# JanEGerken/HEAL-SWIN

Hardware: AMD Instinct MI355X
Metric: images/sec fwd+bwd, HEAL-SWIN nside=256 seg, batch=8 at 1/2/4/8 MI355X (higher is better)
Workload: dtype bf16

## Files before the change

### heal_swin_amd/_lib.py

```python
import ctypes
import os

import numpy as np

_PKG = os.path.dirname(os.path.abspath(__file__))
LIB_PATH = os.path.join(_PKG, "lib", "libhealswin.so")

HS_F32, HS_BF16 = 0, 1
HS_F64 = 3
HS_PRED_LABELS, HS_PRED_ROWS16 = 2, 4
HS_ENSEMBLE_PROB, HS_ENSEMBLE_LOGIT = 0, 1
HS_ATTN_COSINE = 1
HS_ATTN_FORCE_VALU = 2
HS_ATTN_RESIDUAL = 4
HS_ATTN_OVERWRITE_GRADS = 8
HS_EPI_BIAS, HS_EPI_GELU, HS_EPI_DGELU, HS_EPI_RESID = 0, 1, 2, 3
HS_ACC_DEFER = 2
HS_MLP_NORM_AFTER = 16
HS_U8, HS_I32, HS_I64 = 8, 9, 10
HS_FLAT_PATCH_ROWS, HS_FLAT_PIXEL_ROWS, HS_FLAT_IMAGE = 0, 1, 2
HS_DEPTH_L1, HS_DEPTH_L2, HS_DEPTH_HUBER, HS_DEPTH_LOGVAR = 0, 1, 2, 3
HS_DT_NONE, HS_DT_LOG, HS_DT_INV = 0, 1, 2
HS_DT_ZERO_BKG, HS_DT_1000_BKG, HS_DT_AFFINE, HS_DT_INVERSE = 1, 2, 4, 8
HS_DEPTH_STATS_WORDS = 15
HS_HISTOGRAM_MAX_BINS = 4096

c_i64 = ctypes.c_int64
c_int = ctypes.c_int
c_uint = ctypes.c_uint
c_ptr = ctypes.c_void_p
c_float = ctypes.c_float


class WgradProblem(ctypes.Structure):
    _fields_ = [("dy", c_ptr), ("x", c_ptr), ("dw", c_ptr), ("dbias", c_ptr), ("n_out", c_int), ("k_in", c_int), ("accumulate", c_int),
                ("gelu_x", c_int)]


def wgrad_problems(members):
# ... 380 lines not shown
```

### heal_swin_amd/csrc/gemm_nt.hip

```cpp
#include <cstdlib>

#include "hs_gelu.h"

namespace hs {
HS_DEFINE_SEED_EPOCH_SETTER(set_seed_epoch_gemm_nt)

#ifdef HS_GEMM_TRACE
#define HS_GEMM_TRACE_PARAM uint64_t* trace;
constexpr int kTraceCap = 240;
static uint64_t* g_trace = nullptr;
extern "C" int hs_gemm_nt_set_trace(void* buf) {
    g_trace = (uint64_t*)buf;
    return 0;
}
template <typename Params>
void trace_attach(Params& p) {
    p.trace = g_trace;
}
constexpr int trace_lds(int used, int nw) { return used + nw * kTraceCap * 8 <= 163840 ? nw * kTraceCap * 8 : 0; }
struct Trace {
    uint64_t* out;
    bool on;
    int n = 0, nw, wave, lane;
    uint32_t base;
// ... 22 lines not shown
    }
};
#else
#define HS_GEMM_TRACE_PARAM
template <typename Params>
void trace_attach(Params&) {}
constexpr int trace_lds(int, int) { return 0; }
struct Trace {
    template <typename Params>
    __device__ __forceinline__ Trace(const Params&, bool, uint32_t, int, int, int) {}
    __device__ __forceinline__ void operator()(int) const {}
    __device__ __forceinline__ void flush() const {}
};
#endif

namespace {

typedef unsigned int u32x2 __attribute__((__vector_size__(8)));
typedef unsigned int u32x4v __attribute__((__vector_size__(16)));

constexpr int kStoreAux = 2;
constexpr int kInAux = 2;
enum { EPI_BIAS = 0, EPI_GELU = 1, EPI_DGELU = 2, EPI_RESID = 3 };
constexpr int64_t kMaxRecords = 0x7FFFFE00;

struct GemmParams {
    const uint16_t *a, *b;
    int64_t lda, ldb;
    int k;
    const uint16_t *a2, *b2;
    int64_t lda2, ldb2;
    int k2;
    const float* bias;
    uint16_t* c;
    uint16_t* aux;
    int64_t m;
    int n;
    int tiles_n, tiles, per_xcd, blocks_per_xcd;
    float drop_p;
    uint64_t seed;
    HS_GEMM_TRACE_PARAM
};

template <int BM_, int BN_, int WM_, int WN_, int NSTAGE_, bool ALIAS_, int WGS_PER_CU_>
struct TileTraits {
    static constexpr int BM = BM_, BN = BN_, WM = WM_, WN = WN_, NSTAGE = NSTAGE_, WGS_PER_CU = WGS_PER_CU_;
    static constexpr bool ALIAS = ALIAS_;
    static constexpr int NW = WM * WN;
    static constexpr int TM = BM / WM / 32, TN = BN / WN / 32;
    static constexpr int AB = BM * 128, BB = BN * 128, STAGE = AB + BB;
    static constexpr int AHEAD = NSTAGE - 1;
    static_assert(TN == 2 && (TM == 2 || TM == 4), "the kernel is written for wave tiles of 64 columns and 64 or 128 rows");
    static_assert(!ALIAS || NW * 4096 <= STAGE, "patches do not fit a stage buffer");
    static_assert(BN * 4 <= 1024, "a bias slot holds one 1-KB DMA piece");

    static constexpr bool has_in(int epi) { return epi == EPI_DGELU || epi == EPI_RESID; }
    static constexpr bool ring(int epi) { return has_in(epi) && ALIAS && TM == 4 && STAGE >= NW * 8192; }
    static constexpr bool lbias(int epi) { return ALIAS && epi != EPI_DGELU; }
    static constexpr int NSLOT = NSTAGE + 1;
    static constexpr int PATCH_OFF = NSTAGE * STAGE;
    static constexpr int BIAS_OFF = NSTAGE * STAGE + (ALIAS ? 0 : NW * 4096);
    static constexpr int bias_lds(int epi) { return lbias(epi) ? NSLOT * 1024 : 0; }
    static constexpr int trace_off(int epi) { return BIAS_OFF + bias_lds(epi); }
    static constexpr int lds_bytes(int epi) { return trace_off(epi) + trace_lds(trace_off(epi), NW); }
};
using Tile1 = TileTraits<128, 128, 2, 2, 2, false, 2>;
using Tile2 = TileTraits<256, 128, 4, 2, 3, true, 1>;
using Tile3 = TileTraits<256, 256, 2, 4, 2, true, 1>;

constexpr int epi_younger_ops(int tm, int i) {
    const int stores = i < 2 ? i : 1;
    const int last_d = i + 1 < tm - 1 ? i + 1 : tm - 1;
    return 4 * (stores + (last_d - i));
}

template <int OFF>
__device__ __forceinline__ u32x4 lds_read_b128(uint32_t addr) {
    u32x4 v;
    asm volatile("ds_read_b128 %0, %1 offset:%2" : "=v"(v) : "v"(addr), "n"(OFF));
    return v;
}
constexpr int next_in_ring(int x, int n) { return x + 1 == n ? 0 : x + 1; }
__device__ __forceinline__ u32x2 pack_bf16x4(f32x2 lo, f32x2 hi) { return u32x2{pack_bf16x2(lo.x, lo.y), pack_bf16x2(hi.x, hi.y)}; }
__device__ __forceinline__ __amdgpu_buffer_rsrc_t clamped_rsrc(const void* ptr, int64_t bytes) {
    bytes = bytes > kMaxRecords ? kMaxRecords : bytes;
    return __builtin_amdgcn_make_buffer_rsrc((void*)ptr, 0, (int)bytes, 0x00020000);
}
template <int LATER, int EPI_OPS>
__device__ __forceinline__ void wait_pieces_behind() {
    static_assert(LATER + EPI_OPS <= 63, "vmcnt immediate");
    asm volatile("s_waitcnt vmcnt(%0)" ::"n"(LATER + EPI_OPS) : "memory");
}

template <int N_, int LDS_, bool SC>
struct Operand {
    static constexpr int N = N_, LDS = LDS_, J = SC ? 4 : N;
// ... 11 lines not shown
        }
    }
    __device__ __forceinline__ void retarget(const uint16_t* base, int64_t ld, int64_t row0, int64_t rows, int kseg) {
        rsrc = clamped_rsrc(base + row0 * ld, (rows - row0 - 1) * ld * 2 + kseg);
#pragma unroll
        for (int j = 0; j < J; ++j) off[j] = row[j] * ((int)ld * 2) + col[j];
        ld32 = (int)ld * 64;
    }
    __device__ __forceinline__ void issue(unsigned char* stage, int wave, int q, int kb, int kseg) const {
        lds_void* dst = (lds_void*)(stage + LDS + (wave * N + q) * 1024);
        if constexpr (SC) {
            __builtin_amdgcn_raw_ptr_buffer_load_lds(rsrc, dst, 16, (uint32_t)off[q % J], kb + (q >> 2) * ld32, 0, 0);
        } else {
            const uint32_t voff = kb + col[q] < kseg ? (uint32_t)(off[q] + kb) : kOob;
            __builtin_amdgcn_raw_ptr_buffer_load_lds(rsrc, dst, 16, voff, 0, 0, 0);
        }
    }
};
__device__ __forceinline__ uint32_t frag_addr(uint32_t lds_base, int r, int half) {
    const int R = r >> 1;
    return lds_base + R * 256 + (((((r & 1) << 3) + half) ^ (R & 15)) << 4);
}

template <typename Tile, int EPI, bool DROP, bool FAST>
__global__ void __launch_bounds__(Tile::NW * 64, 2) gemm_nt_kernel(GemmParams p) {
#if defined(__HIP_DEVICE_COMPILE__)
    constexpr int BM = Tile::BM, BN = Tile::BN, WM = Tile::WM, WN = Tile::WN, NW = Tile::NW, TM = Tile::TM, TN = Tile::TN;
    constexpr int NSTAGE = Tile::NSTAGE, AHEAD = Tile::AHEAD, NSLOT = Tile::NSLOT, STAGE = Tile::STAGE, BIAS_OFF = Tile::BIAS_OFF;
    constexpr bool ALIAS = Tile::ALIAS, HAS_IN = Tile::has_in(EPI), RING = Tile::ring(EPI), LBIAS = Tile::lbias(EPI);
    constexpr int IW = FAST ? NW / 2 : NW;
    using OperandA = Operand<Tile::AB / 1024 / IW, 0, FAST>;
    using OperandB = Operand<Tile::BB / 1024 / IW, Tile::AB, FAST>;
    constexpr int PIECES = OperandA::N + OperandB::N;
    static_assert(Tile::lds_bytes(EPI) <= 163840, "LDS of one workgroup exceeds 160 KB");
    __shared__ __attribute__((aligned(16))) unsigned char smem[Tile::lds_bytes(EPI)];

    const int tid = threadIdx.x, lane = tid & 63, half = lane >> 5, l31 = lane & 31;
    const int wave = __builtin_amdgcn_readfirstlane(tid >> 6);
    const int wm = wave / WN, wn = wave % WN;

    const int xcd = blockIdx.x & 7, lb = blockIdx.x >> 3;
    const int id_end = min((xcd + 1) * p.per_xcd, p.tiles);
    const int id0 = xcd * p.per_xcd + lb;
    if (id0 >= id_end) return;
    const int nk1 = (p.k + 63) >> 6, nk2 = (p.k2 + 63) >> 6, nk = nk1 + nk2;
    struct Origin {
        int64_t m0;
        int n0;
    };
    auto tile_origin = [&](int id) {
        const int tm = id / p.tiles_n, tn = id - tm * p.tiles_n;
        return Origin{(int64_t)tm * BM, tn * BN};
// ... 86 lines not shown
            constexpr int ks = decltype(ks_c)::value;
            constexpr int rest = PIECES - ks * PQ, cnt = rest < 0 ? 0 : rest < PQ ? rest : PQ;
            wait_frags(ks_c, Int<(ks < 3 ? TM + TN : 0)>{});
            mma(ks_c, Int<ks * PQ>{}, Int<cnt>{});
            if constexpr (ks + 2 < 4) read_frags(Int<ks + 2>{});
        });
    };

    const uint32_t own_rel = wave * 4096 + l31 * 128 + 8 * half;
    const uint32_t own_out_rel = wave * 4096 + l31 * 128 + 8 * (half ^ ((l31 >> 3) & 1));
    const uint32_t row_rel = wave * 4096 + (lane >> 3) * 128 + (((lane & 7) ^ (lane >> 3)) << 4);
    const bool second_half = ((half ^ (lane & (p.n >> 2))) & 1) != 0;
    auto epilogue = [&](int id, int buf_done, int slot_c) {
        const uint32_t patch_off = ALIAS ? buf_done * STAGE : Tile::PATCH_OFF;
        TR(10);
        if (ALIAS) __builtin_amdgcn_s_barrier();
        TR(11);
        const Origin o = tile_origin(id);
        const int64_t m0 = o.m0;
        const int n2 = p.n * 2;
        const int64_t cbytes = (p.m - m0) * (int64_t)n2;
        const __amdgpu_buffer_rsrc_t rc = clamped_rsrc(p.c + m0 * p.n, p.c ? cbytes : 0);
        const __amdgpu_buffer_rsrc_t rx = clamped_rsrc(p.aux + m0 * p.n, p.aux ? cbytes : 0);
        const ElemRng rng(p.drop_p, p.seed);
        const bool wide = RING || (p.n & 7) == 0;
        const int ncol0 = o.n0 + wn * (BN / WN);
        auto col_of = [&](int j, int g) { return ncol0 + j * 32 + 4 * half + 8 * g; };
        float4 bias4[TN][4];
        const uint32_t baddr = lds0 + BIAS_OFF + slot_c * 1024 + (wn * (BN / WN) + 4 * half) * 4;
        auto lds_bias = [&](int j, float4 (&b)[4]) {
            u32x4 bq[4];
#pragma unroll
            for (int g = 0; g < 4; ++g) asm volatile("ds_read_b128 %0, %1" : "=v"(bq[g]) : "v"(baddr + (j * 32 + 8 * g) * 4));
            asm volatile("s_waitcnt lgkmcnt(0)" : "+v"(bq[0]), "+v"(bq[1]), "+v"(bq[2]), "+v"(bq[3]));
#pragma unroll
            for (int g = 0; g < 4; ++g) b[g] = __builtin_bit_cast(float4, bq[g]);
        };
        if constexpr (!LBIAS) {
#pragma unroll
            for (int j = 0; j < TN; ++j)
#pragma unroll
                for (int g = 0; g < 4; ++g) {
                    const int n = col_of(j, g);
                    bias4[j][g] = (EPI != EPI_DGELU && p.bias && n < p.n) ? *(const float4*)(p.bias + n) : make_float4(0.f, 0.f, 0.f, 0.f);
                }
        }
        const int rl_col = ncol0 + (lane & 7) * 8;
        const uint32_t rl_voff = rl_col < p.n ? (uint32_t)((lane >> 3) * n2 + rl_col * 2) : kOob;
        auto row_soff = [&](int i, int t) -> int { return (wm * (BM / WM) + i * 32 + 8 * t) * n2; };
        const int in_col = ncol0 + (((lane & 7) ^ (lane >> 3)) << 3);
        const uint32_t in_voff = in_col < p.n ? (uint32_t)((lane >> 3) * n2 + in_col * 2) : kOob;
        auto request_in = [&](int i) {
            unsigned char* base = smem + patch_off + (i & 1) * (NW * 4096) + wave * 4096;
#pragma unroll
            for (int t = 0; t < 4; ++t)
                __builtin_amdgcn_raw_ptr_buffer_load_lds(rx, (lds_void*)(base + t * 1024), 16, in_voff, row_soff(i, t), 0, kInAux);
        };
        if constexpr (RING) {
            request_in(0);
            request_in(1);
        }
#pragma unroll
        for (int i = 0; i < TM; ++i) {
            const int ml = wm * (BM / WM) + i * 32 + l31;
            auto direct_off = [&](int j, int g) { return col_of(j, g) < p.n ? (uint32_t)(ml * n2 + col_of(j, g) * 2) : kOob; };
            const uint32_t pbase = lds0 + patch_off + (RING ? (i & 1) * (NW * 4096) : 0);
            const uint32_t own_addr = pbase + own_rel, row_addr = pbase + row_rel, own_out = pbase + own_out_rel;
            u32x2 xin[TN][4];
            if (HAS_IN) {
                if (wide) {
                    if constexpr (RING) {
                        static_for<TM>([&](auto b) {
                            if (i == b) asm volatile("s_waitcnt vmcnt(%0)" ::"n"(epi_younger_ops(TM, b)) : "memory");
                        });
                    } else {
                        u32x4 rws[4];
#pragma unroll
                        for (int t = 0; t < 4; ++t)
                            rws[t] = __builtin_bit_cast(u32x4, __builtin_amdgcn_raw_buffer_load_b128(rx, rl_voff, row_soff(i, t), 0));
                        asm volatile("ds_write_b128 %0, %1" ::"v"(row_addr), "v"(rws[0]) : "memory");
                        asm volatile("ds_write_b128 %0, %1 offset:1024" ::"v"(row_addr), "v"(rws[1]) : "memory");
                        asm volatile("ds_write_b128 %0, %1 offset:2048" ::"v"(row_addr), "v"(rws[2]) : "memory");
                        asm volatile("ds_write_b128 %0, %1 offset:3072" ::"v"(row_addr), "v"(rws[3]) : "memory");
                    }
#pragma unroll
                    for (int j = 0; j < TN; ++j)
#pragma unroll
                        for (int g = 0; g < 4; ++g)
                            asm volatile("ds_read_b64 %0, %1" : "=v"(xin[j][g]) : "v"(own_addr + (((4 * j + g) ^ (l31 & 7)) << 4)));
                    asm volatile("s_waitcnt lgkmcnt(0)"
                                 : "+v"(xin[0][0]), "+v"(xin[0][1]), "+v"(xin[0][2]), "+v"(xin[0][3]), "+v"(xin[1][0]),
                                   "+v"(xin[1][1]), "+v"(xin[1][2]), "+v"(xin[1][3]));
                } else {
#pragma unroll
                    for (int j = 0; j < TN; ++j)
#pragma unroll
                        for (int g = 0; g < 4; ++g) xin[j][g] = __builtin_amdgcn_raw_buffer_load_b64(rx, direct_off(j, g), 0, 0);
                }
            }
            auto chunk_key = [&](int j, int g) { return rng.chunk_key((uint64_t)((m0 + ml) * p.n + col_of(j, g)) >> 3); };
            auto keep2 = [&](uint32_t ck, int t) {
                const uint32_t hh = ElemRng::pair_bits(ck, ElemRng::half_mult(second_half, t));
                return f32x2{rng.keep_lo(hh), rng.keep_hi(hh)};
            };
            u32x2 o1[TN][4], o2[TN][4];
#pragma unroll
            for (int j = 0; j < TN; ++j) {
                if constexpr (LBIAS) lds_bias(j, bias4[j]);
#pragma unroll
                for (int g = 0; g < 4; ++g) {
                    f32x16& a16 = acc[j][i];
                    f32x2 v[2] = {f32x2{a16[4 * g], a16[4 * g + 1]} + f32x2{bias4[j][g].x, bias4[j][g].y},
                                  f32x2{a16[4 * g + 2], a16[4 * g + 3]} + f32x2{bias4[j][g].z, bias4[j][g].w}};
                    uint32_t ck = 0;
                    if (DROP) ck = chunk_key(j, g);
// ... 40 lines not shown
                            }
                            o2[j][g] = pack_bf16x4(v[2 * gg], v[2 * gg + 1]);
#pragma unroll
                            for (int r = 0; r < 4; ++r) a16[4 * g + r] = 0.f;
                        }
                    }
            };
            TR(20);
            auto emit = [&](const __amdgpu_buffer_rsrc_t& rs, const u32x2 (&o)[TN][4]) {
                if (wide) {
#pragma unroll
                    for (int j = 0; j < TN; ++j)
#pragma unroll
                        for (int g = 0; g < 4; ++g)
                            asm volatile("ds_write_b64 %0, %1" ::"v"(own_out + (((4 * j + g) ^ (l31 & 7)) << 4)), "v"(o[j][g]) : "memory");
                    u32x4 rws[4];
                    asm volatile("ds_read_b128 %0, %1" : "=v"(rws[0]) : "v"(row_addr));
                    asm volatile("ds_read2_b64 %0, %1 offset0:129 offset1:128" : "=v"(rws[1]) : "v"(row_addr));
                    asm volatile("ds_read_b128 %0, %1 offset:2048" : "=v"(rws[2]) : "v"(row_addr));
                    asm volatile("ds_read2_b64 %0, %1 offset0:129 offset1:128" : "=v"(rws[3]) : "v"(row_addr + 2048));
                    asm volatile("s_waitcnt lgkmcnt(0)" : "+v"(rws[0]), "+v"(rws[1]), "+v"(rws[2]), "+v"(rws[3]));
                    TR(22);
#pragma unroll
                    for (int t = 0; t < 4; ++t)
                        __builtin_amdgcn_raw_buffer_store_b128(__builtin_bit_cast(u32x4v, rws[t]), rs, rl_voff, row_soff(i, t), kStoreAux);
                    asm volatile("s_nop 0" ::"v"(rws[0]), "v"(rws[1]), "v"(rws[2]), "v"(rws[3]));
                } else {
#pragma unroll
                    for (int j = 0; j < TN; ++j)
#pragma unroll
                        for (int g = 0; g < 4; ++g) __builtin_amdgcn_raw_buffer_store_b64(o[j][g], rs, direct_off(j, g), 0, kStoreAux);
                }
            };
            if (EPI == EPI_GELU) {
                if (NW == 8 && wave >= NW / 2) {
                    make_o2();
                    emit(rx, o2);
                    TR(21);
                    __builtin_amdgcn_sched_barrier(0);
                    if (p.c) emit(rc, o1);
                } else {
                    if (p.c) emit(rc, o1);
                    TR(21);
                    __builtin_amdgcn_sched_barrier(0);
                    make_o2();
                    emit(rx, o2);
                }
            } else {
                emit(rc, o1);
            }
            if constexpr (RING) {
                if (i + 2 < TM) request_in(i + 2);
            }
            TR(12 + i);
        }
    };

    const int stride = p.blocks_per_xcd;
    int id_i = id0, ks_i = 0;
    int id_c = id0, ks_c = 0;
    int slot_c = 0;
    auto advance_issue = [&]() {
        ++ks_i;
        if (ks_i == nk) {
            ks_i = 0;
            id_i += stride;
            if (id_i < id_end) retarget(id_i, nk1 == 0, true);
        } else if (ks_i == nk1) {
            retarget(id_i, true, false);
        }
    };
    auto kb_of = [&](int ks) { return (ks >= nk1 ? ks - nk1 : ks) * 128; };
    retarget(id_i, false, true);
    int issued = 0;
#pragma unroll
    for (int q = 0; q < AHEAD; ++q) {
        if (id_i < id_end) {
            issue_pieces(kb_of(ks_i), q, Int<0>{}, Int<PIECES>{});
            advance_issue();
            ++issued;
        }
    }
    int buf = 0, buf_free = AHEAD;
    bool drained = false;
    constexpr int LATER = (AHEAD - 1) * PIECES;
    constexpr int kEpiOps = TM * 4;
    TR(0);
    while (true) {
        TR(3);
        if (IW < NW && wave >= IW) {
        } else if (AHEAD > 1 && issued == AHEAD && !drained)
            wait_pieces_behind<LATER, 0>();
        else if (drained && issued == AHEAD)
            wait_pieces_behind<LATER, kEpiOps>();
        else if (drained && issued == 1)
            wait_pieces_behind<0, kEpiOps>();
        else
            wait_pieces_behind<0, 0>();
        drained = false;
        TR(1);
        __builtin_amdgcn_s_barrier();
        TR(2);
        const bool more = id_i < id_end;
        const bool last = ks_c + 1 == nk;
        compute(buf, more, kb_of(ks_i), buf_free);
        --issued;
        if (more) {
            advance_issue();
            ++issued;
        }
        const int buf_done = buf;
        buf = next_in_ring(buf, NSTAGE);
        buf_free = next_in_ring(buf_free, NSTAGE);
        if (last) {
            epilogue(id_c, buf_done, slot_c);
            slot_c = next_in_ring(slot_c, NSLOT);
            drained = true;
            ks_c = 0;
            id_c += stride;
            if (id_c >= id_end) break;
        } else {
            ++ks_c;
        }
    }
    TR.flush();
#endif
}

template <typename Tile, bool FAST>
int launch_tile(GemmParams& p, int epi, hipStream_t s) {
    const int tiles_m = (int)((p.m + Tile::BM - 1) / Tile::BM);
    p.tiles_n = (p.n + Tile::BN - 1) / Tile::BN;
    const int64_t tiles = (int64_t)tiles_m * p.tiles_n;
    if (tiles > 0x7fffffff) return fail(HS_ERR_UNSUPPORTED, "too many output tiles");
    p.tiles = (int)tiles;
    p.per_xcd = (p.tiles + 7) / 8;
    const int resident = usable_cus_per_xcd() * Tile::WGS_PER_CU;
    p.blocks_per_xcd = p.per_xcd < resident ? p.per_xcd : resident;
    const dim3 grid((unsigned)(8 * p.blocks_per_xcd)), block(Tile::NW * 64);
    using Kernel = void (*)(GemmParams);
    static constexpr Kernel kKernels[4][2] = {
        {gemm_nt_kernel<Tile, EPI_BIAS, false, FAST>, gemm_nt_kernel<Tile, EPI_BIAS, false, FAST>},
        {gemm_nt_kernel<Tile, EPI_GELU, false, FAST>, gemm_nt_kernel<Tile, EPI_GELU, true, FAST>},
        {gemm_nt_kernel<Tile, EPI_DGELU, false, FAST>, gemm_nt_kernel<Tile, EPI_DGELU, true, FAST>},
        {gemm_nt_kernel<Tile, EPI_RESID, false, FAST>, gemm_nt_kernel<Tile, EPI_RESID, false, FAST>}};
    hipLaunchKernelGGL(kKernels[epi][p.drop_p > 0.f], grid, block, 0, s, p);
    HS_LAUNCH_CHECK("gemm_nt");
    return HS_OK;
}

}

int gemm_nt_check_shape(const char* who, int64_t lda, int64_t ldb, int k, int64_t lda2, int64_t ldb2, int k2, int64_t m, int n) {
    HS_CHECK_ARG(m > 0 && n > 0 && k > 0 && k2 >= 0, "%s: empty shape", who);
    if (k % 8 || k2 % 8 || lda % 8 || ldb % 8 || (k2 && (lda2 % 8 || ldb2 % 8)) || n % 4)
        return fail(HS_ERR_UNSUPPORTED, "%s: k, k2 and the row strides must be multiples of 8, n a multiple of 4", who);
    if (lda * 2 * 256 > kMaxRecords || ldb * 2 * 256 > kMaxRecords || (int64_t)n * 2 * 256 > kMaxRecords)
        return fail(HS_ERR_UNSUPPORTED, "%s: row stride too large", who);
    if (((m + 127) / 128) * (((int64_t)n + 127) / 128) > 0x7fffffff) return fail(HS_ERR_UNSUPPORTED, "%s: too many output tiles", who);
    return HS_OK;
}

int gemm_nt_tile_variant(int forced, int64_t m, int n, int k, int k2, int epilogue) {
    int variant = forced;
    if (!variant) {
        const int64_t tiles2 = ((m + 255) / 256) * ((n + 127) / 128), tiles3 = ((m + 255) / 256) * ((n + 255) / 256);
        if (tiles2 < 256)
            variant = 1;
        else if ((epilogue == EPI_GELU || epilogue == EPI_DGELU) ? n >= 512 : (n >= 1024 && k + k2 >= 512))
// ... 1 lines not shown
        else if (n >= 256 && tiles3 >= 768 && k % 64 == 0 && k2 % 64 == 0)
            variant = 3;
        else
            variant = 2;
    }
    if (variant == 3 && (epilogue == EPI_DGELU || epilogue == EPI_RESID) && n % 8) variant = 2;
    return variant == 2 || variant == 3 ? variant : 1;
}

}

namespace {
int g_tile_variant = 0;
}

extern "C" {

int hs_gemm_nt_set_tile(int variant) {
    g_tile_variant = variant;
    return HS_OK;
}

int hs_gemm_nt_tile_variant(int64_t m, int n, int k, int k2, int epilogue) {
    return hs::gemm_nt_tile_variant(g_tile_variant, m, n, k, k2, epilogue);
}

int hs_gemm_nt(const void* a, int64_t lda, const void* b, int64_t ldb, int k, const void* a2, int64_t lda2, const void* b2,
               int64_t ldb2, int k2, const float* bias, void* c, void* aux, int64_t m, int n, int epilogue, float drop_p,
               uint64_t seed, int dtype, void* stream) {
    using namespace hs;
    HS_CHECK_ARG(dtype == HS_BF16, "hs_gemm_nt: bf16 activations only (fp32 runs use the library GEMM)");
    HS_CHECK_ARG(a && b && m > 0 && n > 0 && k > 0, "hs_gemm_nt: null operand or empty shape");
    HS_CHECK_ARG(epilogue >= EPI_BIAS && epilogue <= EPI_RESID, "hs_gemm_nt: unknown epilogue %d", epilogue);
    HS_CHECK_ARG(k2 == 0 || (a2 && b2 && k2 > 0), "hs_gemm_nt: second segment needs a2, b2, k2 > 0");
    HS_CHECK_ARG(c || (epilogue == EPI_GELU && aux), "hs_gemm_nt: no output");
    HS_CHECK_ARG(epilogue == EPI_BIAS || aux, "hs_gemm_nt: this epilogue needs aux");
    HS_CHECK_ARG(drop_p >= 0.f && drop_p <= 1.f, "hs_gemm_nt: drop_p must be in [0, 1]");
    HS_CHECK_ALIGNED("hs_gemm_nt", 16, a, b, a2, b2, bias, c, aux);
    if (int st = gemm_nt_check_shape("hs_gemm_nt", lda, ldb, k, lda2, ldb2, k2, m, n)) return st;
    GemmParams p{};
    p.a = (const uint16_t*)a; p.b = (const uint16_t*)b; p.lda = lda; p.ldb = ldb; p.k = k;
    p.a2 = (const uint16_t*)a2; p.b2 = (const uint16_t*)b2; p.lda2 = lda2; p.ldb2 = ldb2; p.k2 = k2;
    p.bias = bias; p.c = (uint16_t*)c; p.aux = (uint16_t*)aux; p.m = m; p.n = n;
    p.drop_p = drop_p; p.seed = seed;
    trace_attach(p);
    hipStream_t st = (hipStream_t)stream;
    const bool fast = k % 64 == 0 && k2 % 64 == 0;
    switch (gemm_nt_tile_variant(g_tile_variant, m, n, k, k2, epilogue)) {
        case 2: return fast ? launch_tile<Tile2, true>(p, epilogue, st) : launch_tile<Tile2, false>(p, epilogue, st);
        case 3: return fast ? launch_tile<Tile3, true>(p, epilogue, st) : launch_tile<Tile3, false>(p, epilogue, st);
        default: return launch_tile<Tile1, false>(p, epilogue, st);
    }
}

}
```

### heal_swin_amd/ops/gemm.py

```python
import math
import os

import torch

from .. import _lib
from .._lib import check, lib, ptr, stream_ptr
from . import runtime
from .runtime import RT, _aligned, _cast_param, _defer_flag, _defer_keep, _require_gpu, _sink_buffer, _timed


OWN_GEMM = os.environ.get("HS_OWN_GEMM", "auto")


OWN_GELU_MAX_K = 4096
OWN_DGELU_MAX_K = 1024
OWN_BIAS_MAX_K = 0


class GemmTuner:
    MIN_FLOP = 1 << 33

    def __init__(self):
        self.picks = {}
        self.trials = {}
# ... 54 lines not shown
    if epi == _lib.HS_EPI_DGELU:
        return kk <= OWN_DGELU_MAX_K
    if epi == _lib.HS_EPI_GELU:
        return kk <= OWN_GELU_MAX_K
    if OWN_BIAS_MAX_K > 0:
        return kk <= OWN_BIAS_MAX_K
    if GEMM_TUNE and m is not None and k2 == 0 and torch.cuda.is_available():
        pick = GEMM_TUNER.pick(int(m), n, kk, torch.device("cuda", torch.cuda.current_device()))
        if pick is not None:
            return pick
    return kk <= 128 or n <= 128 or (n <= 256 and kk <= 256)


RESID_DGRAD_OWN = True


def own_gemm_legal(n, k, dtype):
    return dtype == torch.bfloat16 and OWN_GEMM != "0" and k % 8 == 0 and n % 8 == 0 and n >= 16


RESID_EPILOGUE = True


def gemm_nt(a2d, w, bias=None, epi=0, aux=None, a2=None, w2=None, want_c=True, drop_p=0.0, seed=0):
    w, w2, bias = _aligned(w), _aligned(w2), _aligned(bias)
    if epi != _lib.HS_EPI_GELU:
        aux = _aligned(aux)
    m, k = a2d.shape
    n = w.shape[0]
    assert a2d.stride(1) == 1 and w.stride(1) == 1 and a2d.dtype == torch.bfloat16 and w.dtype == torch.bfloat16
    c = torch.empty((m, n), dtype=torch.bfloat16, device=a2d.device) if want_c else None
    if epi == _lib.HS_EPI_GELU:
        aux = torch.empty((m, n), dtype=torch.bfloat16, device=a2d.device)
    k2 = 0 if a2 is None else a2.shape[1]
    if bias is not None and bias.dtype != torch.float32:
        bias = bias.float()
    with _timed(f"hs_gemm_nt epi={epi} m={m} n={n} k={k + k2}", a2d.device, 2 * (m * (k + k2) + n * (k + k2) + m * n * (2 if (epi and want_c) else 1)), 2 * m * n * (k + k2)):
        check(lib.hs_gemm_nt(ptr(a2d), a2d.stride(0), ptr(w), w.stride(0), k, ptr(a2), 0 if a2 is None else a2.stride(0), ptr(w2),
                             0 if w2 is None else w2.stride(0), k2, ptr(bias), ptr(c), ptr(aux), m, n, epi, float(drop_p), int(seed),
                             _lib.HS_BF16, stream_ptr(a2d.device)), "hs_gemm_nt")
    return c, aux


def _lib_tag(kind, m, n, k):
    return f"lib {kind} m={m} n={n} k={k}"


FP32_GEMM = os.environ.get("HS_FP32_GEMM", "bf16x3")
_BF16X3_MIN = 160
_SPLIT_MEMO = []
_MM_OUT_DTYPE = [None]


def _bf16x3_ok(x, n=None, k=None):
    ok = FP32_GEMM == "bf16x3" and x.dtype == torch.float32 and x.is_cuda and x.shape[-1] % 8 == 0
    ok = ok and (n is None or n * k >= _BF16X3_MIN * (n + k))
    if ok and _MM_OUT_DTYPE[0] is None:
        _probe_mm_out_dtype(x.device)
    return ok and _MM_OUT_DTYPE[0] is not False


def _probe_mm_out_dtype(device):
# ... 396 lines not shown
```

### heal_swin_amd/ops/mlp_branch.py

```python
import os

import torch

from .. import _lib
from .._lib import check, lib, ptr, stream_ptr
from .runtime import RT, _aligned, _cast_param, _defer_flag, _defer_keep, _draw_seed, _extras, _f32, _require_gpu, _timed
from .norm import _norm_param_grads, _norm_param_result
from .gemm import (_Split, _bf16x3_ok, _cast_param_t, _input_grad, _lib_linear, _lib_linear_resid, _lib_matmul, _param_grads, lib_resid_ok, _split_of, gemm_nt, own_gemm_legal, own_gemm_ok)


class MlpFn(torch.autograd.Function):

    @staticmethod
    def forward(ctx, x, w1, b1, w2, b2, drop_p, seed, passthrough, residual=None):
        _require_gpu(x, w1, b1, w2, b2, residual)
        c_in, hid = w1.shape[1], w1.shape[0]
        x2 = x.reshape(-1, c_in)
        if not x2.is_contiguous():
            x2 = x2.contiguous()
        dt = x.dtype
        x3 = a3 = None
        w1c, w2c = _cast_param(w1, dt), _cast_param(w2, dt)
        need_grad = any(ctx.needs_input_grad[:5])
        if own_gemm_ok(_lib.HS_EPI_GELU, hid, c_in, dt):
            h, a = gemm_nt(x2, w1c, b1, _lib.HS_EPI_GELU, want_c=need_grad, drop_p=drop_p, seed=seed)
        else:
            h = _lib_linear(x2, w1c, None if b1 is None else _cast_param(b1, dt))
            x3 = _split_of(x2)
            if _bf16x3_ok(h, w2.shape[0], hid) and w2c.dtype == torch.float32 and w2.shape[0] % 8 == 0 and hid % 8 == 0:
                h = _aligned(h)
                a3 = torch.empty((h.shape[0], 3 * hid), dtype=torch.bfloat16, device=h.device)
                check(lib.hs_gelu_split3(None, ptr(h), ptr(a3), h.shape[0], hid, float(drop_p), int(seed), stream_ptr(h.device)),
                      "hs_gelu_split3")
                a = _Split(a3, hid)
            else:
                a = torch.empty_like(h)
                check(lib.hs_gelu_fwd(ptr(h), ptr(a), h.numel(), float(drop_p), int(seed), _lib.dtype_code(dt), stream_ptr(h.device)),
                      "hs_gelu_fwd")
        ctx.has_residual = residual is not None
        res2 = None
        if residual is not None:
            res2 = residual.reshape(-1, w2.shape[0])
            res2 = res2 if res2.is_contiguous() else res2.contiguous()
        lib_res = res2 is not None and lib_resid_ok(w2.shape[0], hid, dt) and not own_gemm_ok(_lib.HS_EPI_BIAS, w2.shape[0], hid, dt, m=x2.shape[0])
        if lib_res:
            y = _lib_linear_resid(a, w2c, None if b2 is None else _cast_param(b2, dt), res2)
        elif res2 is not None and own_gemm_legal(w2.shape[0], hid, dt):
            y = gemm_nt(a, w2c, b2, _lib.HS_EPI_RESID, aux=res2)[0]
# ... 9 lines not shown
        assert not isinstance(a, _Split)
        ctx.save_for_backward(None if x3 is not None else x2, h, None if a3 is not None else a, w1, w2)
        ctx.biases = (b1, b2)
        ctx.casts = (w1c if w1c.dtype != w1.dtype else None, w2c if w2c.dtype != w2.dtype else None)
        ctx.cast_cache = RT.cast_cache
        ctx.meta = (float(drop_p), int(seed), x.shape)
        ctx.splits = (x3, a3)
        y = y.view(x.shape[:-1] + (w2.shape[0],))
        return (y, x.view_as(x)) if passthrough else y

    @staticmethod
    def backward(ctx, dy, dx_res=None):
        x2, h, a, w1, w2 = ctx.saved_tensors
        b1, b2 = ctx.biases
        w1c, w2c = ctx.casts
        p, seed, xshape = ctx.meta
        if dy is None:
            return dx_res, None, None, None, None, None, None, None, None
        c_out, hid, c_in = w2.shape[0], w1.shape[0], w1.shape[1]
        dy2 = dy.reshape(-1, c_out)
        if not dy2.is_contiguous():
            dy2 = dy2.contiguous()
        dt = dy2.dtype
        if own_gemm_ok(_lib.HS_EPI_DGELU, hid, c_out, dt):
            dh = gemm_nt(dy2, _cast_param_t(w2, dt, ctx.cast_cache), None, _lib.HS_EPI_DGELU, aux=h, drop_p=p, seed=seed)[0]
        else:
            da = _lib_matmul(dy2, w2c if (w2c is not None and w2c.dtype == dt) else w2.to(dt))
            if _bf16x3_ok(da, c_in, hid) and w1.dtype == torch.float32 and c_in % 8 == 0 and hid % 8 == 0:
                dh3 = torch.empty((h.shape[0], 3 * hid), dtype=torch.bfloat16, device=h.device)
                check(lib.hs_gelu_split3(ptr(_aligned(da)), ptr(_aligned(h)), ptr(dh3), h.shape[0], hid, p, seed, stream_ptr(h.device)), "hs_gelu_split3")
                dh = _Split(dh3, hid)
            else:
                dh = torch.empty_like(h)
                check(lib.hs_gelu_bwd(ptr(da), ptr(h), ptr(dh), h.numel(), p, seed, _lib.dtype_code(dt), stream_ptr(h.device)), "hs_gelu_bwd")
            del da
        dx = None
        if ctx.needs_input_grad[0]:
            dx = _input_grad(dh, w1, w1c, None if dx_res is None else dx_res.reshape(-1, c_in), ctx.cast_cache).reshape(xshape)
        ctx.casts = ctx.cast_cache = None
        (x3, a3), ctx.splits = ctx.splits, (None, None)
        dw2, db2 = _param_grads(dy2, a, w2, b2, ctx.needs_input_grad[3], b2 is not None and ctx.needs_input_grad[4], a3)
        dw1, db1 = _param_grads(dh, x2, w1, b1, ctx.needs_input_grad[1], b1 is not None and ctx.needs_input_grad[2], x3)
        return dx, dw1, db1, dw2, db2, None, None, None, (dy if ctx.has_residual else None)


def mlp(x, w1, b1, w2, b2, drop_p=0.0, seed=None, passthrough=False, residual=None):
    if drop_p > 0.0 and seed is None:
        seed = _draw_seed()
# ... 122 lines not shown
```

### include/healswin.h

```cpp
#ifndef HEALSWIN_H
#define HEALSWIN_H

#include <stdint.h>

#ifdef __cplusplus
extern "C" {
#endif

typedef enum {
    HS_OK = 0,
    HS_ERR_INVALID_ARG = 1,
    HS_ERR_UNSUPPORTED = 2,
    HS_ERR_HIP = 3,
    HS_ERR_NOT_PERMUTATION = 4,
    HS_ERR_MISALIGNED = 5
} hs_status;

typedef enum { HS_F32 = 0, HS_BF16 = 1 } hs_dtype;

#define HS_ATTN_COSINE 1u
#define HS_ATTN_FORCE_VALU 2u
#define HS_ATTN_RESIDUAL 4u
#define HS_ATTN_OVERWRITE_GRADS 8u

// ... 205 lines not shown
                              int64_t n_tokens, int channels, int num_heads, int window_size, unsigned flags, int dtype,
                              void* stream);

int hs_window_attn_module_fwd_train(const void* x, void* out, void* xn_out, float* mean_out, float* rstd_out, void* qkv_out,
                                    void* attn_out, float* lse_out, const void* qkv_w, const float* qkv_b, const void* proj_w,
                                    const float* proj_b, const float* ln_gamma, const float* ln_beta, const float* bias,
                                    const float* head_scale, const int32_t* idx, int64_t roll, const uint8_t* labels,
                                    const float* norm2_gamma, const float* norm2_beta, void* n2_out, float* mean2_out, float* rstd2_out,
                                    int batch, int64_t n_tokens, int channels, int num_heads, int window_size, unsigned flags, int dtype,
                                    void* stream);

int64_t hs_window_attn_module_bwd_chain_workspace(int batch, int64_t n_tokens, int channels, int num_heads, int window_size);
int hs_window_attn_module_bwd_chain(const void* dout, const void* x, const void* xn, const float* mean, const float* rstd, const void* qkv,
                              const void* attn_out, const float* lse, const void* qkv_w_t, const void* proj_w_t, const float* ln_gamma,
                              const float* bias, const float* head_scale, const int32_t* idx, int64_t roll, const uint8_t* labels,
                              void* dx, float* dqkv_w, float* dqkv_b, float* dproj_w, float* dproj_b, float* dln_gamma, float* dln_beta,
                              float* dbias, float* dhead_scale, float* workspace, int accumulate, int batch, int64_t n_tokens, int channels,
                              int num_heads, int window_size, unsigned flags, int dtype, void* stream);

#define HS_EPI_BIAS 0
#define HS_EPI_GELU 1
#define HS_EPI_DGELU 2
#define HS_EPI_RESID 3
int hs_gemm_nt(const void* a, int64_t lda, const void* b, int64_t ldb, int k, const void* a2, int64_t lda2, const void* b2,
               int64_t ldb2, int k2, const float* bias, void* c, void* aux, int64_t m, int n, int epilogue, float drop_p,
               uint64_t seed, int dtype, void* stream);
int hs_gemm_nt_set_tile(int variant);
int hs_gemm_nt_tile_variant(int64_t m, int n, int k, int k2, int epilogue);

int hs_lib_gemm_supported(void);
int hs_lib_gemm_set_supported(int on);
int hs_lib_gemm_nt(const void* a, const void* w, const void* bias, int bias_dtype, const void* c, void* d, int64_t m, int n, int k,
                   void* stream);
int hs_lib_gemm_pick(int64_t m, int n, int k, int has_c, int* index, int* solution, char* name, int name_len);
int hs_lib_gemm_set_pick(int64_t m, int n, int k, int has_c, int index);

int hs_pix2ang_nest(int nside, int64_t first, int64_t count, double* theta, double* phi);
int hs_sample_bilinear_u8(const void* img, int batch, int channels, int height, int width, const double* rx, const double* ry,
                          int64_t n, void* out, void* stream);
int hs_sample_mask_u8(const void* mask, int batch, int height, int width, const double* rx, const double* ry, int64_t n,
                      int background, void* out, void* stream);

typedef struct hs_fisheye_camera {
    double k[8];
    double cx_offset, cy_offset, aspect_ratio;
    int poly_order, width, height;
// ... 223 lines not shown
```

Before: 58.82.

## Store MLP hidden activations as per-tile records for the GELU-backward GEMM

Adds an HS_EPI_RECORDS mode for the 256x256 tile. The forward GELU GEMM writes the pre-activation h in a tile-blocked record layout that follows the per-wave fragment order, so each lane stores contiguous 16-byte chunks. The backward DGELU GEMM reads those records straight into LDS and skips the swizzled per-row segment reads and the stride-dependent addressing. It is on by default through HS_MLP_RECORDS. In exchange, h becomes an opaque padded buffer tied to the forward and backward GEMMs both picking tile variant 3.

```diff
diff --git a/heal_swin_amd/_lib.py b/heal_swin_amd/_lib.py
--- a/heal_swin_amd/_lib.py
+++ b/heal_swin_amd/_lib.py
@@ -15,6 +15,7 @@
 HS_ATTN_RESIDUAL = 4
 HS_ATTN_OVERWRITE_GRADS = 8
 HS_EPI_BIAS, HS_EPI_GELU, HS_EPI_DGELU, HS_EPI_RESID = 0, 1, 2, 3
+HS_EPI_RECORDS = 0x100
 HS_ACC_DEFER = 2
 HS_MLP_NORM_AFTER = 16
 HS_U8, HS_I32, HS_I64 = 8, 9, 10
diff --git a/heal_swin_amd/csrc/gemm_nt.hip b/heal_swin_amd/csrc/gemm_nt.hip
--- a/heal_swin_amd/csrc/gemm_nt.hip
+++ b/heal_swin_amd/csrc/gemm_nt.hip
@@ -68,6 +68,8 @@
 constexpr int kStoreAux = 2;
 constexpr int kInAux = 2;
 enum { EPI_BIAS = 0, EPI_GELU = 1, EPI_DGELU = 2, EPI_RESID = 3 };
+enum { EPI_CODE_MASK = 0xff, EPI_RECORDS = 0x100 };
+constexpr int kRowOps = 4;
 constexpr int64_t kMaxRecords = 0x7FFFFE00;
 
 struct GemmParams {
@@ -103,6 +105,8 @@
     static constexpr bool has_in(int epi) { return epi == EPI_DGELU || epi == EPI_RESID; }
     static constexpr bool ring(int epi) { return has_in(epi) && ALIAS && TM == 4 && STAGE >= NW * 8192; }
     static constexpr bool lbias(int epi) { return ALIAS && epi != EPI_DGELU; }
+    static constexpr bool records(int epi) { return ALIAS && TM == 4 && NW == 8 && (epi == EPI_GELU || epi == EPI_DGELU); }
+    static constexpr int RECORD = BM * BN;
     static constexpr int NSLOT = NSTAGE + 1;
     static constexpr int PATCH_OFF = NSTAGE * STAGE;
     static constexpr int BIAS_OFF = NSTAGE * STAGE + (ALIAS ? 0 : NW * 4096);
@@ -117,7 +121,7 @@
 constexpr int epi_younger_ops(int tm, int i) {
     const int stores = i < 2 ? i : 1;
     const int last_d = i + 1 < tm - 1 ? i + 1 : tm - 1;
-    return 4 * (stores + (last_d - i));
+    return kRowOps * (stores + (last_d - i));
 }
 
 template <int OFF>
@@ -175,12 +179,13 @@
     return lds_base + R * 256 + (((((r & 1) << 3) + half) ^ (R & 15)) << 4);
 }
 
-template <typename Tile, int EPI, bool DROP, bool FAST>
+template <typename Tile, int EPI, bool DROP, bool FAST, bool REC = false>
 __global__ void __launch_bounds__(Tile::NW * 64, 2) gemm_nt_kernel(GemmParams p) {
 #if defined(__HIP_DEVICE_COMPILE__)
     constexpr int BM = Tile::BM, BN = Tile::BN, WM = Tile::WM, WN = Tile::WN, NW = Tile::NW, TM = Tile::TM, TN = Tile::TN;
     constexpr int NSTAGE = Tile::NSTAGE, AHEAD = Tile::AHEAD, NSLOT = Tile::NSLOT, STAGE = Tile::STAGE, BIAS_OFF = Tile::BIAS_OFF;
     constexpr bool ALIAS = Tile::ALIAS, HAS_IN = Tile::has_in(EPI), RING = Tile::ring(EPI), LBIAS = Tile::lbias(EPI);
+    static_assert(!REC || (Tile::records(EPI) && (EPI == EPI_GELU || RING)), "records: the 256 x 256 tile's GELU / GELU' epilogues");
     constexpr int IW = FAST ? NW / 2 : NW;
     using OperandA = Operand<Tile::AB / 1024 / IW, 0, FAST>;
     using OperandB = Operand<Tile::BB / 1024 / IW, Tile::AB, FAST>;
@@ -313,6 +318,9 @@
         const int64_t cbytes = (p.m - m0) * (int64_t)n2;
         const __amdgpu_buffer_rsrc_t rc = clamped_rsrc(p.c + m0 * p.n, p.c ? cbytes : 0);
         const __amdgpu_buffer_rsrc_t rx = clamped_rsrc(p.aux + m0 * p.n, p.aux ? cbytes : 0);
+        uint16_t* const hrec = EPI == EPI_GELU ? p.c : p.aux;
+        const __amdgpu_buffer_rsrc_t rrec = clamped_rsrc(hrec + (REC ? (int64_t)id * Tile::RECORD : 0), REC && hrec ? Tile::RECORD * 2 : 0);
+        auto rec_soff = [&](int i, int t) -> int { return wave * (TM * kRowOps * 1024) + (i * kRowOps + t) * 1024; };
         const ElemRng rng(p.drop_p, p.seed);
         const bool wide = RING || (p.n & 7) == 0;
         const int ncol0 = o.n0 + wn * (BN / WN);
@@ -344,8 +352,10 @@
         auto request_in = [&](int i) {
             unsigned char* base = smem + patch_off + (i & 1) * (NW * 4096) + wave * 4096;
 #pragma unroll
-            for (int t = 0; t < 4; ++t)
-                __builtin_amdgcn_raw_ptr_buffer_load_lds(rx, (lds_void*)(base + t * 1024), 16, in_voff, row_soff(i, t), 0, kInAux);
+            for (int t = 0; t < kRowOps; ++t) {
+                if constexpr (REC) __builtin_amdgcn_raw_ptr_buffer_load_lds(rrec, (lds_void*)(base + t * 1024), 16, lane * 16, rec_soff(i, t), 0, kInAux);
+                else __builtin_amdgcn_raw_ptr_buffer_load_lds(rx, (lds_void*)(base + t * 1024), 16, in_voff, row_soff(i, t), 0, kInAux);
+            }
         };
         if constexpr (RING) {
             request_in(0);
@@ -374,14 +384,26 @@
                         asm volatile("ds_write_b128 %0, %1 offset:2048" ::"v"(row_addr), "v"(rws[2]) : "memory");
                         asm volatile("ds_write_b128 %0, %1 offset:3072" ::"v"(row_addr), "v"(rws[3]) : "memory");
                     }
-#pragma unroll
-                    for (int j = 0; j < TN; ++j)
-#pragma unroll
-                        for (int g = 0; g < 4; ++g)
-                            asm volatile("ds_read_b64 %0, %1" : "=v"(xin[j][g]) : "v"(own_addr + (((4 * j + g) ^ (l31 & 7)) << 4)));
-                    asm volatile("s_waitcnt lgkmcnt(0)"
-                                 : "+v"(xin[0][0]), "+v"(xin[0][1]), "+v"(xin[0][2]), "+v"(xin[0][3]), "+v"(xin[1][0]),
-                                   "+v"(xin[1][1]), "+v"(xin[1][2]), "+v"(xin[1][3]));
+                    if constexpr (REC) {
+                        const uint32_t rec_addr = pbase + wave * 4096 + lane * 16;
+                        u32x4 r[kRowOps] = {lds_read_b128<0>(rec_addr), lds_read_b128<1024>(rec_addr), lds_read_b128<2048>(rec_addr),
+                                            lds_read_b128<3072>(rec_addr)};
+                        asm volatile("s_waitcnt lgkmcnt(0)" : "+v"(r[0]), "+v"(r[1]), "+v"(r[2]), "+v"(r[3]));
+#pragma unroll
+                        for (int t = 0; t < kRowOps; ++t) {
+                            xin[t / 2][2 * (t % 2)] = u32x2{r[t].x, r[t].y};
+                            xin[t / 2][2 * (t % 2) + 1] = u32x2{r[t].z, r[t].w};
+                        }
+                    } else {
+#pragma unroll
+                        for (int j = 0; j < TN; ++j)
+#pragma unroll
+                            for (int g = 0; g < 4; ++g)
+                                asm volatile("ds_read_b64 %0, %1" : "=v"(xin[j][g]) : "v"(own_addr + (((4 * j + g) ^ (l31 & 7)) << 4)));
+                        asm volatile("s_waitcnt lgkmcnt(0)"
+                                     : "+v"(xin[0][0]), "+v"(xin[0][1]), "+v"(xin[0][2]), "+v"(xin[0][3]), "+v"(xin[1][0]),
+                                       "+v"(xin[1][1]), "+v"(xin[1][2]), "+v"(xin[1][3]));
+                    }
                 } else {
 #pragma unroll
                     for (int j = 0; j < TN; ++j)
@@ -468,7 +490,7 @@
                     asm volatile("s_waitcnt lgkmcnt(0)" : "+v"(rws[0]), "+v"(rws[1]), "+v"(rws[2]), "+v"(rws[3]));
                     TR(22);
 #pragma unroll
-                    for (int t = 0; t < 4; ++t)
+                    for (int t = 0; t < kRowOps; ++t)
                         __builtin_amdgcn_raw_buffer_store_b128(__builtin_bit_cast(u32x4v, rws[t]), rs, rl_voff, row_soff(i, t), kStoreAux);
                     asm volatile("s_nop 0" ::"v"(rws[0]), "v"(rws[1]), "v"(rws[2]), "v"(rws[3]));
                 } else {
@@ -478,15 +500,30 @@
                         for (int g = 0; g < 4; ++g) __builtin_amdgcn_raw_buffer_store_b64(o[j][g], rs, direct_off(j, g), 0, kStoreAux);
                 }
             };
+            auto emit_h = [&]() {
+                if constexpr (REC) {
+                    u32x4v rws[kRowOps];
+#pragma unroll
+                    for (int t = 0; t < kRowOps; ++t) {
+                        const u32x2 lo = o1[t / 2][2 * (t % 2)], hi = o1[t / 2][2 * (t % 2) + 1];
+                        rws[t] = u32x4v{lo[0], lo[1], hi[0], hi[1]};
+                        __builtin_amdgcn_raw_buffer_store_b128(rws[t], rrec, lane * 16, rec_soff(i, t), kStoreAux);
+                    }
+                    asm volatile("s_nop 0" ::"v"(rws[0]), "v"(rws[1]), "v"(rws[2]), "v"(rws[3]));
+                } else {
+                    emit(rc, o1);
+                }
+            };
+            static_assert(TN * 4 >= kRowOps, "the direct form stores no fewer instructions than the row-segment form");
             if (EPI == EPI_GELU) {
                 if (NW == 8 && wave >= NW / 2) {
                     make_o2();
                     emit(rx, o2);
                     TR(21);
                     __builtin_amdgcn_sched_barrier(0);
-                    if (p.c) emit(rc, o1);
+                    if (p.c) emit_h();
                 } else {
-                    if (p.c) emit(rc, o1);
+                    if (p.c) emit_h();
                     TR(21);
                     __builtin_amdgcn_sched_barrier(0);
                     make_o2();
@@ -530,7 +567,7 @@
     int buf = 0, buf_free = AHEAD;
     bool drained = false;
     constexpr int LATER = (AHEAD - 1) * PIECES;
-    constexpr int kEpiOps = TM * 4;
+    constexpr int kEpiOps = TM * kRowOps;
     TR(0);
     while (true) {
         TR(3);
@@ -574,7 +611,7 @@
 }
 
 template <typename Tile, bool FAST>
-int launch_tile(GemmParams& p, int epi, hipStream_t s) {
+int launch_tile(GemmParams& p, int epi, bool records, hipStream_t s) {
     const int tiles_m = (int)((p.m + Tile::BM - 1) / Tile::BM);
     p.tiles_n = (p.n + Tile::BN - 1) / Tile::BN;
     const int64_t tiles = (int64_t)tiles_m * p.tiles_n;
@@ -590,7 +627,18 @@
         {gemm_nt_kernel<Tile, EPI_GELU, false, FAST>, gemm_nt_kernel<Tile, EPI_GELU, true, FAST>},
         {gemm_nt_kernel<Tile, EPI_DGELU, false, FAST>, gemm_nt_kernel<Tile, EPI_DGELU, true, FAST>},
         {gemm_nt_kernel<Tile, EPI_RESID, false, FAST>, gemm_nt_kernel<Tile, EPI_RESID, false, FAST>}};
-    hipLaunchKernelGGL(kKernels[epi][p.drop_p > 0.f], grid, block, 0, s, p);
+    Kernel kernel = kKernels[epi][p.drop_p > 0.f];
+    if (records) {
+        if constexpr (Tile::records(EPI_GELU) && Tile::ring(EPI_DGELU)) {
+            static constexpr Kernel kRecords[2][2] = {
+                {gemm_nt_kernel<Tile, EPI_GELU, false, FAST, true>, gemm_nt_kernel<Tile, EPI_GELU, true, FAST, true>},
+                {gemm_nt_kernel<Tile, EPI_DGELU, false, FAST, true>, gemm_nt_kernel<Tile, EPI_DGELU, true, FAST, true>}};
+            kernel = kRecords[epi == EPI_DGELU][p.drop_p > 0.f];
+        } else {
+            return fail(HS_ERR_UNSUPPORTED, "hs_gemm_nt: HS_EPI_RECORDS needs the 256 x 256 tile (ask hs_gemm_nt_tile_variant)");
+        }
+    }
+    hipLaunchKernelGGL(kernel, grid, block, 0, s, p);
     HS_LAUNCH_CHECK("gemm_nt");
     return HS_OK;
 }
@@ -638,7 +686,7 @@
 }
 
 int hs_gemm_nt_tile_variant(int64_t m, int n, int k, int k2, int epilogue) {
-    return hs::gemm_nt_tile_variant(g_tile_variant, m, n, k, k2, epilogue);
+    return hs::gemm_nt_tile_variant(g_tile_variant, m, n, k, k2, epilogue & hs::EPI_CODE_MASK);
 }
 
 int hs_gemm_nt(const void* a, int64_t lda, const void* b, int64_t ldb, int k, const void* a2, int64_t lda2, const void* b2,
@@ -647,7 +695,11 @@
     using namespace hs;
     HS_CHECK_ARG(dtype == HS_BF16, "hs_gemm_nt: bf16 activations only (fp32 runs use the library GEMM)");
     HS_CHECK_ARG(a && b && m > 0 && n > 0 && k > 0, "hs_gemm_nt: null operand or empty shape");
+    const bool records = (epilogue & EPI_RECORDS) != 0;
+    HS_CHECK_ARG(!(epilogue & ~(EPI_CODE_MASK | EPI_RECORDS)), "hs_gemm_nt: unknown epilogue flags %#x", epilogue);
+    epilogue &= EPI_CODE_MASK;
     HS_CHECK_ARG(epilogue >= EPI_BIAS && epilogue <= EPI_RESID, "hs_gemm_nt: unknown epilogue %d", epilogue);
+    HS_CHECK_ARG(!records || epilogue == EPI_GELU || epilogue == EPI_DGELU, "hs_gemm_nt: HS_EPI_RECORDS goes with HS_EPI_GELU / _DGELU");
     HS_CHECK_ARG(k2 == 0 || (a2 && b2 && k2 > 0), "hs_gemm_nt: second segment needs a2, b2, k2 > 0");
     HS_CHECK_ARG(c || (epilogue == EPI_GELU && aux), "hs_gemm_nt: no output");
     HS_CHECK_ARG(epilogue == EPI_BIAS || aux, "hs_gemm_nt: this epilogue needs aux");
@@ -663,10 +715,10 @@
     hipStream_t st = (hipStream_t)stream;
     const bool fast = k % 64 == 0 && k2 % 64 == 0;
     switch (gemm_nt_tile_variant(g_tile_variant, m, n, k, k2, epilogue)) {
-        case 2: return fast ? launch_tile<Tile2, true>(p, epilogue, st) : launch_tile<Tile2, false>(p, epilogue, st);
-        case 3: return fast ? launch_tile<Tile3, true>(p, epilogue, st) : launch_tile<Tile3, false>(p, epilogue, st);
-        default: return launch_tile<Tile1, false>(p, epilogue, st);
-    }
-}
-
-}
+        case 2: return fast ? launch_tile<Tile2, true>(p, epilogue, records, st) : launch_tile<Tile2, false>(p, epilogue, records, st);
+        case 3: return fast ? launch_tile<Tile3, true>(p, epilogue, records, st) : launch_tile<Tile3, false>(p, epilogue, records, st);
+        default: return launch_tile<Tile1, false>(p, epilogue, records, st);
+    }
+}
+
+}
diff --git a/heal_swin_amd/ops/gemm.py b/heal_swin_amd/ops/gemm.py
--- a/heal_swin_amd/ops/gemm.py
+++ b/heal_swin_amd/ops/gemm.py
@@ -100,7 +100,18 @@
 RESID_EPILOGUE = True
 
 
-def gemm_nt(a2d, w, bias=None, epi=0, aux=None, a2=None, w2=None, want_c=True, drop_p=0.0, seed=0):
+RECORD_ELEMS = 256 * 256
+
+
+def record_elems(m, n):
+    return -(-m // 256) * -(-n // 256) * RECORD_ELEMS
+
+
+def records_ok(m, n, k, k2=0):
+    return all(lib.hs_gemm_nt_tile_variant(int(m), int(n), int(kk), 0, e) == 3 for kk, e in ((k, _lib.HS_EPI_GELU), (k2 or k, _lib.HS_EPI_DGELU)))
+
+
+def gemm_nt(a2d, w, bias=None, epi=0, aux=None, a2=None, w2=None, want_c=True, drop_p=0.0, seed=0, records=False):
     w, w2, bias = _aligned(w), _aligned(w2), _aligned(bias)
     if epi != _lib.HS_EPI_GELU:
         aux = _aligned(aux)
@@ -108,6 +119,14 @@
     n = w.shape[0]
     assert a2d.stride(1) == 1 and w.stride(1) == 1 and a2d.dtype == torch.bfloat16 and w.dtype == torch.bfloat16
     c = torch.empty((m, n), dtype=torch.bfloat16, device=a2d.device) if want_c else None
+    flags = 0
+    if records:
+        assert epi in (_lib.HS_EPI_GELU, _lib.HS_EPI_DGELU)
+        flags = _lib.HS_EPI_RECORDS
+        if epi == _lib.HS_EPI_DGELU:
+            assert aux.dtype == torch.bfloat16 and aux.is_contiguous() and aux.numel() == record_elems(m, n)
+        elif want_c:
+            c = torch.empty(record_elems(m, n), dtype=torch.bfloat16, device=a2d.device)
     if epi == _lib.HS_EPI_GELU:
         aux = torch.empty((m, n), dtype=torch.bfloat16, device=a2d.device)
     k2 = 0 if a2 is None else a2.shape[1]
@@ -115,7 +134,7 @@
         bias = bias.float()
     with _timed(f"hs_gemm_nt epi={epi} m={m} n={n} k={k + k2}", a2d.device, 2 * (m * (k + k2) + n * (k + k2) + m * n * (2 if (epi and want_c) else 1)), 2 * m * n * (k + k2)):
         check(lib.hs_gemm_nt(ptr(a2d), a2d.stride(0), ptr(w), w.stride(0), k, ptr(a2), 0 if a2 is None else a2.stride(0), ptr(w2),
-                             0 if w2 is None else w2.stride(0), k2, ptr(bias), ptr(c), ptr(aux), m, n, epi, float(drop_p), int(seed),
+                             0 if w2 is None else w2.stride(0), k2, ptr(bias), ptr(c), ptr(aux), m, n, epi | flags, float(drop_p), int(seed),
                              _lib.HS_BF16, stream_ptr(a2d.device)), "hs_gemm_nt")
     return c, aux
 
diff --git a/heal_swin_amd/ops/mlp_branch.py b/heal_swin_amd/ops/mlp_branch.py
--- a/heal_swin_amd/ops/mlp_branch.py
+++ b/heal_swin_amd/ops/mlp_branch.py
@@ -6,7 +6,10 @@
 from .._lib import check, lib, ptr, stream_ptr
 from .runtime import RT, _aligned, _cast_param, _defer_flag, _defer_keep, _draw_seed, _extras, _f32, _require_gpu, _timed
 from .norm import _norm_param_grads, _norm_param_result
-from .gemm import (_Split, _bf16x3_ok, _cast_param_t, _input_grad, _lib_linear, _lib_linear_resid, _lib_matmul, _param_grads, lib_resid_ok, _split_of, gemm_nt, own_gemm_legal, own_gemm_ok)
+from .gemm import (_Split, _bf16x3_ok, _cast_param_t, _input_grad, _lib_linear, _lib_linear_resid, _lib_matmul, _param_grads, lib_resid_ok, _split_of, gemm_nt, own_gemm_legal, own_gemm_ok, records_ok)
+
+
+MLP_RECORDS = os.environ.get("HS_MLP_RECORDS", "1") != "0"
 
 
 class MlpFn(torch.autograd.Function):
@@ -22,8 +25,11 @@
         x3 = a3 = None
         w1c, w2c = _cast_param(w1, dt), _cast_param(w2, dt)
         need_grad = any(ctx.needs_input_grad[:5])
+        ctx.h_records = False
         if own_gemm_ok(_lib.HS_EPI_GELU, hid, c_in, dt):
-            h, a = gemm_nt(x2, w1c, b1, _lib.HS_EPI_GELU, want_c=need_grad, drop_p=drop_p, seed=seed)
+            ctx.h_records = bool(MLP_RECORDS and need_grad and own_gemm_ok(_lib.HS_EPI_DGELU, hid, w2.shape[0], dt) and
+                                 records_ok(x2.shape[0], hid, c_in, w2.shape[0]))
+            h, a = gemm_nt(x2, w1c, b1, _lib.HS_EPI_GELU, want_c=need_grad, drop_p=drop_p, seed=seed, records=ctx.h_records)
         else:
             h = _lib_linear(x2, w1c, None if b1 is None else _cast_param(b1, dt))
             x3 = _split_of(x2)
@@ -79,8 +85,9 @@
         if not dy2.is_contiguous():
             dy2 = dy2.contiguous()
         dt = dy2.dtype
-        if own_gemm_ok(_lib.HS_EPI_DGELU, hid, c_out, dt):
-            dh = gemm_nt(dy2, _cast_param_t(w2, dt, ctx.cast_cache), None, _lib.HS_EPI_DGELU, aux=h, drop_p=p, seed=seed)[0]
+        if ctx.h_records or own_gemm_ok(_lib.HS_EPI_DGELU, hid, c_out, dt):
+            dh = gemm_nt(dy2, _cast_param_t(w2, dt, ctx.cast_cache), None, _lib.HS_EPI_DGELU, aux=h, drop_p=p, seed=seed,
+                         records=ctx.h_records)[0]
         else:
             da = _lib_matmul(dy2, w2c if (w2c is not None and w2c.dtype == dt) else w2.to(dt))
             if _bf16x3_ok(da, c_in, hid) and w1.dtype == torch.float32 and c_in % 8 == 0 and hid % 8 == 0:
diff --git a/include/healswin.h b/include/healswin.h
--- a/include/healswin.h
+++ b/include/healswin.h
@@ -251,6 +251,7 @@
 #define HS_EPI_GELU 1
 #define HS_EPI_DGELU 2
 #define HS_EPI_RESID 3
+#define HS_EPI_RECORDS 0x100
 int hs_gemm_nt(const void* a, int64_t lda, const void* b, int64_t ldb, int k, const void* a2, int64_t lda2, const void* b2,
                int64_t ldb2, int k2, const float* bias, void* c, void* aux, int64_t m, int n, int epilogue, float drop_p,
                uint64_t seed, int dtype, void* stream);
```

Result: no change. 58.96 (median of 6 runs) (+0.2%).
